# seanwood/gcc-nmf

Measured on AMD Instinct MI355X. Metric: stereo frames/sec (1024-FFT, K=1024, 100 NMF iters), higher is better.
Workload: dtype f32; 1 GPU; HBM-resident (float32 samples in HBM -> separated float32 waveforms in HBM; the host-to-host rates are the host_to_host_* fields of a --full run): 64 x 10 s stereo @16 kHz synthetic mixtures per GPU (SURVEY 8d recipe), 1024-pt FFT hop 256 (F=513, T=622/file), K=1024, 100 KL-NMF iters, 128 TDOAs, 3 targets, independent dictionary per file; dictionary_size=1024, parallelism=file-sharded x1, no data-path collective

## Files before the change

### gcc_nmf_amd/csrc/gemm_dma.h

```cpp
#pragma once
#include <mutex>
#include <type_traits>
#include "gemm_mfma.h"
#include "chain_sync.h"

#ifndef GEMM_DMA_ABL
#define GEMM_DMA_ABL 0
#endif

typedef __attribute__((address_space(3))) void* gemm_lds_ptr;
typedef __attribute__((address_space(1))) const void* gemm_glb_ptr;

__device__ __forceinline__ void gemm_dma16(const float* wave_uniform_base, unsigned lane_byte_offset, unsigned lds_wave_byte_addr) {
    asm volatile("s_mov_b32 m0, %2\n\tglobal_load_lds_dwordx4 %0, %1"
                 :
                 : "v"(lane_byte_offset), "s"(wave_uniform_base), "s"(lds_wave_byte_addr)
                 : "memory");
}

__device__ __forceinline__ void gemm_dma16_masked(const float* wave_uniform_base, unsigned lane_byte_offset, unsigned lds_wave_byte_addr,
                                                  unsigned long long wave_uniform_mask) {
    unsigned long long saved;
    asm volatile("s_mov_b64 %0, exec\n\ts_mov_b64 exec, %4\n\ts_mov_b32 m0, %3\n\tglobal_load_lds_dwordx4 %1, %2\n\ts_mov_b64 exec, %0"
                 : "=&s"(saved)
// ... 8 lines not shown
__device__ __forceinline__ gemm_f32x4 gemm_lds_read_b128(unsigned byte_addr) {
    gemm_f32x4 v;
    asm volatile("ds_read_b128 %0, %1 offset:%2" : "=v"(v) : "v"(byte_addr), "n"(OFF));
    return v;
}
typedef float gemm_f32x2 __attribute__((ext_vector_type(2)));
template <int OFF0, int OFF1>
__device__ __forceinline__ gemm_f32x2 gemm_lds_read2_b32(unsigned byte_addr) {
    gemm_f32x2 v;
    asm volatile("ds_read2_b32 %0, %1 offset0:%2 offset1:%3" : "=v"(v) : "v"(byte_addr), "n"(OFF0), "n"(OFF1));
    return v;
}

__device__ __forceinline__ void gemm_wait_lds() { asm volatile("s_waitcnt lgkmcnt(0)" ::: "memory"); }
template <typename T>
__device__ __forceinline__ void gemm_tie(T& v) { asm volatile("" : "+v"(v)); }

__device__ __forceinline__ void gemm_barrier_arrive(unsigned counter_byte_addr) {
    unsigned long long saved;
    asm volatile("s_mov_b64 %0, exec\n\ts_mov_b64 exec, 1\n\tds_add_u32 %1, %2\n\ts_mov_b64 exec, %0"
                 : "=&s"(saved)
                 : "v"(counter_byte_addr), "v"(1u)
                 : "memory");
}
__device__ __forceinline__ unsigned gemm_barrier_peek(unsigned counter_byte_addr) {
    unsigned seen;
    asm volatile("ds_read_b32 %0, %1" : "=v"(seen) : "v"(counter_byte_addr) : "memory");
    return seen;
}
__device__ __forceinline__ void gemm_barrier_wait(unsigned counter_byte_addr, unsigned target, unsigned seen) {
    unsigned seen_s;
    asm volatile("s_waitcnt lgkmcnt(0)\n1:\n\tv_readfirstlane_b32 %1, %0\n\ts_cmp_ge_u32 %1, %3\n\ts_cbranch_scc1 2f\n\t"
                 "s_sleep 1\n\tds_read_b32 %0, %2\n\ts_waitcnt lgkmcnt(0)\n\ts_branch 1b\n2:"
                 : "+v"(seen), "=&s"(seen_s)
                 : "v"(counter_byte_addr), "s"(target)
                 : "memory", "scc");
}

template <bool KC, int NT, int ROWS>
struct GemmFrag;
template <int NT, int ROWS>
struct GemmFrag<true, NT, ROWS> {
    gemm_f32x4 v[NT];
    __device__ __forceinline__ void read(unsigned base) {
        v[0] = gemm_lds_read_b128<0 * 2048>(base);
        v[1] = gemm_lds_read_b128<1 * 2048>(base);
        if constexpr (NT == 4) {
            v[2] = gemm_lds_read_b128<2 * 2048>(base);
            v[3] = gemm_lds_read_b128<3 * 2048>(base);
        }
    }
    __device__ __forceinline__ void tie() {
// ... 100 lines not shown
                } else {
#pragma unroll
                    for (int r = 0; r < 16; ++r) u[r] = gemm_div_fast(x[r], u[r]);
                }
            }
#pragma unroll
            for (int r = 0; r < 16; ++r) gemm_buffer_store(u[r], C, lane_off, ro + ((r & 3) + 8 * (r >> 2)) * rstep, 0);
        };
        if (oka) column(acc_a, xa, ba, lo);
        if (okb) column(acc_b, xb, bb, lo + 128);
    }
};

template <bool TAIL>
__device__ __forceinline__ void gemm_epilogue_update_w_full(const GemmArgs& p, int file, int col0, int tid, int wm, int l31, int hh,
                                                            bool wave_active, f32x16 (&acc)[4][2], float tail_acc, float rowsum_acc,
                                                            float* smem) {
    float* s_rs = smem;
    float* s_tail = smem + 64;
    float* s_red = smem + 320;
    float* s_norm = smem + 640;
    float rs = rowsum_acc;
    rs += __shfl_xor(rs, 1);
    rs += __shfl_xor(rs, 2);
    if ((tid & 3) == 0) s_rs[tid >> 2] = rs;
    if (TAIL) s_tail[tid] = tail_acc;
    __syncthreads();
    const int ca = l31, cb = l31 + 32;
    const float ira = 1.0f / s_rs[ca], irb = 1.0f / s_rs[cb];
    const gemm_i32x4 W = gemm_buffer_rsrc(p.C + file * p.sC);
    const int lo = 4 * (4 * hh * p.ldc + col0 + l31), rstep = 4 * p.ldc;
    float ssa = 0.f, ssb = 0.f;
    if (wave_active) {
#pragma unroll
        for (int m = 0; m < 4; ++m) {
            const int ro = (wm * 128 + m * 32) * rstep;
            float wa[16], wb[16];
#pragma unroll
            for (int r = 0; r < 16; ++r) {
                const int so = ro + ((r & 3) + 8 * (r >> 2)) * rstep;
// ... 157 lines not shown
        const int r = t - (len + s), base_r = list * p.cr;
        const int lenr = min(max(p.batch * p.rag * p.tiles_m - base_r, 0), p.cr);
        if (r >= lenr) return false;
        const int idx = base_r + r;
        q = idx / p.tiles_m;
        tm = idx - q * p.tiles_m;
        col0 = (p.tiles_n - 1) * 64;
        nw = 1;
    }
    file = gemm_dma_list_file(p, q) + p.file0;
    return true;
}

template <int TM>
struct GemmDmaLds {
    static constexpr int SBUF = 128 * TM * 16 + 64 * 16 + 16 + 16;
};

template <bool A_KC, bool B_KC, int EPI, bool TAIL, int TM, bool NARROW>
__device__ __forceinline__ void gemm_dma_workgroup(const GemmArgs& p, float* const smem, float* const s_rowvec, unsigned* const s_arrivals_p,
                                                   const int list, const int t, const GemmSync& sync, const int sync_it = 0,
                                                   const bool trace_on = true) {
    static_assert(TM == 4 || TM == 2, "");
    static_assert(TM == 4 || EPI != EPI_UPDW, "the fused W update owns all rows of its atoms: full-height tiles only");
    static_assert(!NARROW || (EPI != EPI_UPDW && TM == 4), "narrow items: full-height tiles with an element-wise epilogue");
    constexpr int BK = 16, BM = 128 * TM, BN = 64, RW = 32 * TM;
    constexpr int NA = 2 * TM;
    constexpr int SA = BM * BK, SB = BN * BK;
    constexpr int SBUF = SA + SB + BK + BK;
    static_assert(SBUF == GemmDmaLds<TM>::SBUF, "");
    constexpr bool SCALE = !B_KC && (EPI == EPI_DIV || EPI == EPI_STORE);
    unsigned& s_arrivals = *s_arrivals_p;

    const int tid = threadIdx.x, lane = tid & 63;
    const int wave = __builtin_amdgcn_readfirstlane(tid >> 6);
    const int wm = wave, wn = 0;
    const int l31 = lane & 31, hh = lane >> 5;

    int nkt = (p.Kd + BK - 1) / BK;
    int n_item = p.N;
    int n_sync = p.N;
    int file = 0, tm = 0, col0 = 0, nw = 2, row0 = 0;
    const float* __restrict__ A = nullptr;
    const float* __restrict__ B = nullptr;
    const float* __restrict__ bscale = nullptr;
    const float* __restrict__ tail_src = nullptr;
    const float* __restrict__ scale_src = nullptr;
    unsigned long long tail_mask = 0, scale_mask = 0;
    bool wave_active = false, do_tail = false, do_rowsum = false;
    unsigned offA[NA], offB = 0;
    auto take_item = [&]() -> bool {
        int f_, tm_, c_, nw_;
        if (!gemm_dma_item(p, list, t, f_, tm_, c_, nw_)) return false;
        file = __builtin_amdgcn_readfirstlane(f_);
        tm = __builtin_amdgcn_readfirstlane(tm_);
        col0 = __builtin_amdgcn_readfirstlane(c_);
        nw = NARROW ? __builtin_amdgcn_readfirstlane(nw_) : 2;
        if (p.ragged_n) {
            const int nf = __builtin_amdgcn_readfirstlane(p.ragged_n[file]);
            n_sync = nf;
            if (p.ragged_kd) nkt = (nf + BK - 1) / BK;
            else n_item = nf;
        }
        row0 = tm * BM;
        A = p.A + file * p.sA;
        B = p.B + file * p.sB;
        bscale = (SCALE && p.bscale) ? p.bscale + file * p.s_bscale : nullptr;
        wave_active = (row0 + wm * RW) < p.M;
        do_tail = TAIL && (tm == 0);
        do_rowsum = B_KC && (p.rowsumB != nullptr || EPI == EPI_UPDW) && (tm == 0);
        tail_src = A + (long)p.tail_row * p.lda;
        tail_mask = (wave == 0 && do_tail) ? 0x0full : 0ull;
        scale_mask = (wave == 0 && bscale != nullptr) ? 0xf0ull : 0ull;
        scale_src = bscale != nullptr ? bscale : A;
        return true;
    };
    auto set_offsets = [&]() {
#pragma unroll
        for (int i = 0; i < NA; ++i) {
            const int piece = wave * NA + i;
            if (A_KC) {
                const int row = piece * 16 + (lane >> 2), c = (lane & 3) ^ gemm_swz(piece * 16 + (lane >> 2));
                offA[i] = 4u * (unsigned)(min(row0 + row, p.a_clamp) * p.lda + 4 * c);
            } else {
                constexpr int PPR = BM / 256;
                const int kk = piece / PPR, col = (piece % PPR) * 256 + lane * 4;
                offA[i] = 4u * (unsigned)(kk * p.lda + min(row0 + col, p.a_clamp));
            }
        }
        if (B_KC) {
            const int row = wave * 16 + (lane >> 2), c = (lane & 3) ^ gemm_swz(row);
            offB = 4u * (unsigned)(min(col0 + row, p.b_clamp) * p.ldb + 4 * c);
        } else {
            const int kk = wave * 4 + (lane >> 4), col = (lane & 15) * 4;
            offB = 4u * (unsigned)(kk * p.ldb + min(col0 + col, p.b_clamp));
        }
    };

    f32x16 acc[TM][2];
    float tail_acc = 0.f, rowsum_acc = 0.f;

    const unsigned lds0 = __builtin_amdgcn_readfirstlane((unsigned)(size_t)(gemm_lds_ptr)smem);
    unsigned side_off = 0;

    auto dma_piece = [&](const int piece, const int kt, const int buf) {
#ifdef GEMM_DMA_SKIP_FROM
        if (piece >= GEMM_DMA_SKIP_FROM) return;
#endif
        if (piece < NA) {
            gemm_dma16(A + (A_KC ? (long)kt * BK : (long)kt * BK * p.lda), offA[piece], lds0 + 4 * (buf * SBUF + (wave * NA + piece) * 256));
        } else if (piece == NA) {
            gemm_dma16(B + (B_KC ? (long)kt * BK : (long)kt * BK * p.ldb), offB, lds0 + 4 * (buf * SBUF + SA + wave * 256));
        } else {
            if (TAIL || SCALE) {
                const unsigned dst = lds0 + 4 * (buf * SBUF + SA + SB);
                if (TAIL) gemm_dma16_masked(tail_src + kt * BK, side_off, dst, tail_mask);
                if (SCALE) gemm_dma16_masked(scale_src + kt * BK, side_off, dst, scale_mask);
            }
        }
    };
    constexpr int NPIECES = NA + 2;
#ifdef GEMM_DMA_SPREAD
    constexpr int SPREAD = GEMM_DMA_SPREAD;
#else
    constexpr int SPREAD = (A_KC && !B_KC) ? 1 : 2;
#endif

    const gemm_f32x4 zero4 = {0.f, 0.f, 0.f, 0.f};
    GemmFrag<A_KC, TM, BM> a0, a1;
    GemmFrag<B_KC, 2, BN> b0, b1;
    gemm_f32x4 sc0 = zero4, sc1 = zero4, t4 = zero4, tb4 = zero4, ts4 = zero4, rs4 = zero4;
    gemm_f32x2 tbxy = {0.f, 0.f}, tbzw = {0.f, 0.f};

    const unsigned arrivals_addr = (unsigned)(size_t)(gemm_lds_ptr)s_arrivals_p;
    unsigned oA0 = 0, oA1 = 0, oB0 = 0, oB1 = 0, oTB = 0, oRS = 0;
    const int tg = wave;
    auto set_lane_constants = [&]() {
        const int arow = wm * RW + l31, bcol = wn * 64 + l31, tj = lane;
        side_off = 16u * (unsigned)(lane & 3);
        oA0 = A_KC ? 4 * (arow * 16 + 4 * ((0 + hh) ^ gemm_swz(arow))) : 4 * (4 * (0 + hh) * BM + arow);
        oA1 = A_KC ? 4 * (arow * 16 + 4 * ((2 + hh) ^ gemm_swz(arow))) : 4 * (4 * (2 + hh) * BM + arow);
        oB0 = 4 * SA + (B_KC ? 4 * (bcol * 16 + 4 * ((0 + hh) ^ gemm_swz(bcol))) : 4 * (4 * (0 + hh) * BN + bcol));
        oB1 = 4 * SA + (B_KC ? 4 * (bcol * 16 + 4 * ((2 + hh) ^ gemm_swz(bcol))) : 4 * (4 * (2 + hh) * BN + bcol));
        oTB = 4 * SA + (B_KC ? 4 * (tj * 16 + 4 * (tg ^ gemm_swz(tj))) : 4 * (4 * tg * BN + tj));
        oRS = 4 * SA + 4 * ((tid >> 2) * 16 + 4 * (tid & 3));
    };

    auto read_group0 = [&](const unsigned lds) {
        if (wave_active) {
            a0.read(lds + oA0);
            b0.read(lds + oB0);
        }
        if (SCALE) sc0 = gemm_lds_read_b128<4 * (SA + SB + BK)>(lds + 16 * hh);
    };
    auto read_group1 = [&](const unsigned lds) {
        if (wave_active) {
            a1.read(lds + oA1);
            b1.read(lds + oB1);
        }
        if (SCALE) sc1 = gemm_lds_read_b128<4 * (SA + SB + BK) + 32>(lds + 16 * hh);
        if (TAIL) {
            t4 = gemm_lds_read_b128<4 * (SA + SB)>(lds + 16 * tg);
            if (B_KC) {
                tb4 = gemm_lds_read_b128<0>(lds + oTB);
            } else {
                tbxy = gemm_lds_read2_b32<0 * BN, 1 * BN>(lds + oTB);
                tbzw = gemm_lds_read2_b32<2 * BN, 3 * BN>(lds + oTB);
                if (SCALE) ts4 = gemm_lds_read_b128<4 * (SA + SB + BK)>(lds + 16 * tg);
            }
        }
        if (B_KC) rs4 = gemm_lds_read_b128<0>(lds + oRS);
    };
    auto wait_group0 = [&]() {
        gemm_wait_lds();
        a0.tie();
        b0.tie();
        if (SCALE) {
            gemm_tie(sc0);
            b0.scale(sc0);
        }
    };
    auto wait_group1 = [&]() {
        gemm_wait_lds();
        a1.tie();
        b1.tie();
        if (SCALE) {
            gemm_tie(sc1);
            b1.scale(sc1);
        }
        if (TAIL) {
            gemm_tie(t4);
            if (B_KC) {
                gemm_tie(tb4);
            } else {
                gemm_tie(tbxy);
                gemm_tie(tbzw);
                tb4 = gemm_f32x4{tbxy.x, tbxy.y, tbzw.x, tbzw.y};
                if (SCALE) {
                    gemm_tie(ts4);
                    tb4 *= ts4;
                }
            }
        }
        if (B_KC) gemm_tie(rs4);
    };
    auto mma = [&](auto nw_c, const GemmFrag<A_KC, TM, BM>& a, const GemmFrag<B_KC, 2, BN>& b, const int e, const int m) {
        constexpr int NW = decltype(nw_c)::value;
        acc[m][0] = __builtin_amdgcn_mfma_f32_32x32x2f32(a.get(m, e), b.get(0, e), acc[m][0], 0, 0, 0);
        if constexpr (NW == 2) acc[m][1] = __builtin_amdgcn_mfma_f32_32x32x2f32(a.get(m, e), b.get(1, e), acc[m][1], 0, 0, 0);
    };

#ifdef GEMM_DMA_PROBE
    unsigned long long probe[7] = {0, 0, 0, 0, 0, 0, 0};
#define GEMM_PROBE(i_) const unsigned long long pt##i_ = __builtin_amdgcn_s_memtime()
#define GEMM_PROBE_DECL(i_) unsigned long long pt##i_ = 0
#define GEMM_PROBE_SET(i_) pt##i_ = __builtin_amdgcn_s_memtime()
#else
#define GEMM_PROBE(i_)
#define GEMM_PROBE_DECL(i_)
#define GEMM_PROBE_SET(i_)
#endif
    auto step = [&](auto cur_c, auto nw_c, const int kt) {
        constexpr int CUR = decltype(cur_c)::value;
        const unsigned ldsC = lds0 + 4 * CUR * SBUF, ldsN = lds0 + 4 * (CUR ^ 1) * SBUF;
        const int ktn = min(kt + 1, nkt - 1);
        GEMM_PROBE(0);
#if !(GEMM_DMA_ABL & 1)
        read_group1(ldsC);
#endif
        __builtin_amdgcn_sched_barrier(0);
        if (wave_active) {
            if (SPREAD == 0) {
#pragma unroll
                for (int i = 0; i < NPIECES; ++i) dma_piece(i, ktn, CUR ^ 1);
                __builtin_amdgcn_sched_barrier(0);
            }
#pragma unroll
            for (int e = 0; e < 4; ++e)
#pragma unroll
                for (int m = 0; m < TM; ++m) {
                    mma(nw_c, a0, b0, e, m);
                    const int slot = e * TM + m;
                    if (SPREAD == 1 && slot < NPIECES) {
                        dma_piece(slot, ktn, CUR ^ 1);
                        __builtin_amdgcn_sched_barrier(0);
                    }
                    if (SPREAD == 2 && slot % 3 != 2 && (slot / 3) * 2 + slot % 3 < NPIECES) {
                        dma_piece((slot / 3) * 2 + slot % 3, ktn, CUR ^ 1);
                        __builtin_amdgcn_sched_barrier(0);
                    }
                }
        } else {
#pragma unroll
            for (int i = 0; i < NPIECES; ++i) dma_piece(i, ktn, CUR ^ 1);
        }
        __builtin_amdgcn_sched_barrier(0);
        GEMM_PROBE(1);
        wait_group1();
        GEMM_PROBE(2);
        GEMM_PROBE_DECL(3);
        GEMM_PROBE_DECL(4);
        GEMM_PROBE_DECL(5);
        unsigned seen = 0;
#ifndef GEMM_DMA_ARRIVE_E
#define GEMM_DMA_ARRIVE_E 1
#define GEMM_DMA_WAIT_E 3
#endif
#pragma unroll
        for (int e = 0; e < 4; ++e) {
            if (e == GEMM_DMA_ARRIVE_E) {
                __builtin_amdgcn_sched_barrier(0);
                GEMM_PROBE_SET(3);
                asm volatile("s_waitcnt vmcnt(0)" ::: "memory");
#if !(GEMM_DMA_ABL & 2)
                gemm_barrier_arrive(arrivals_addr);
#endif
                __builtin_amdgcn_sched_barrier(0);
            }
            if (e == GEMM_DMA_WAIT_E - 1) {
                __builtin_amdgcn_sched_barrier(0);
#if !(GEMM_DMA_ABL & 2)
                seen = gemm_barrier_peek(arrivals_addr);
#endif
                __builtin_amdgcn_sched_barrier(0);
            }
            if (e == GEMM_DMA_WAIT_E) {
                __builtin_amdgcn_sched_barrier(0);
                GEMM_PROBE_SET(4);
#if !(GEMM_DMA_ABL & 2)
                gemm_barrier_wait(arrivals_addr, 4u * (unsigned)(kt + 1), seen);
#endif
                GEMM_PROBE_SET(5);
#if !(GEMM_DMA_ABL & 1)
                read_group0(ldsN);
#endif
                __builtin_amdgcn_sched_barrier(0);
            }
            if (wave_active) {
#pragma unroll
                for (int m = 0; m < TM; ++m) mma(nw_c, a1, b1, e, m);
            }
        }
        if (TAIL) {
            tail_acc = fmaf(t4.x, tb4.x, tail_acc);
            tail_acc = fmaf(t4.y, tb4.y, tail_acc);
            tail_acc = fmaf(t4.z, tb4.z, tail_acc);
            tail_acc = fmaf(t4.w, tb4.w, tail_acc);
        }
        if (B_KC) rowsum_acc += (rs4.x + rs4.y) + (rs4.z + rs4.w);
        __builtin_amdgcn_sched_barrier(0);
        GEMM_PROBE(6);
        wait_group0();
#ifdef GEMM_DMA_PROBE
        __builtin_amdgcn_sched_barrier(0);
        const unsigned long long pt7 = __builtin_amdgcn_s_memtime();
        probe[0] += pt1 - pt0;
        probe[1] += pt2 - pt1;
        probe[2] += pt3 - pt2;
        probe[3] += pt4 - pt3;
        probe[4] += pt5 - pt4;
        probe[5] += pt6 - pt5;
        probe[6] += pt7 - pt6;
        __builtin_amdgcn_sched_barrier(0);
#endif
    };
    auto main_loop = [&](auto nw_c) {
        for (int kt = 0; kt < nkt; kt += 2) {
            step(std::integral_constant<int, 0>{}, nw_c, kt);
            if (kt + 1 < nkt) step(std::integral_constant<int, 1>{}, nw_c, kt + 1);
        }
    };

    if (SCALE) {
        if (!p.bscale && tid < 2 * BK) smem[(tid >> 4) * SBUF + SA + SB + BK + (tid & 15)] = 1.f;
    }
    bool have = take_item();
    if (have) set_offsets();
    long long* trace_row = nullptr;
    while (have) {
        const int vb = p.lists == 8 ? 8 * t + list : t;
        trace_row = (trace_on && p.trace && vb < p.trace_rows) ? p.trace + 8 * (long)vb : nullptr;
        if (trace_row && tid == 0) {
            trace_row[0] = trace_row[1] = __builtin_amdgcn_s_memrealtime();
            trace_row[4] = (long long)((__builtin_amdgcn_s_getreg((3 << 11) | 20) & 15u) << 16 | (__builtin_amdgcn_s_getreg((31 << 11) | 4) & 0xffffu));
            trace_row[7] = (long long)blockIdx.x << 16;
        }
        set_lane_constants();
        gemm_sync_wait(sync, file, col0, tid, sync_it, list, n_sync);
        if (trace_row && tid == 0) trace_row[1] = __builtin_amdgcn_s_memrealtime();
#pragma unroll
        for (int i = 0; i < NPIECES; ++i) dma_piece(i, 0, 0);
#pragma unroll
        for (int m = 0; m < TM; ++m)
#pragma unroll
            for (int n = 0; n < 2; ++n)
#pragma unroll
                for (int r = 0; r < 16; ++r) acc[m][n][r] = 0.f;
        tail_acc = 0.f;
        rowsum_acc = 0.f;
        if constexpr (EPI == EPI_STORE || EPI == EPI_UPDH) {
#pragma unroll
            for (int i = 0; i < BM / 256; ++i) {
                const int lr = tid + 256 * i, row = min(row0 + lr, p.M - 1);
                s_rowvec[lr] = p.ktailA ? p.ktailA[file * p.s_ktailA + row] : 0.f;
                if (EPI == EPI_UPDH) {
                    const float rd = 1.0f / (p.E2[file * p.sE2 + row] + p.alpha + p.eps);
                    s_rowvec[BM + lr] = p.E1 ? p.E1[file * p.sE1 + row] * rd : rd;
                }
            }
        }
        if (tid == 0) s_arrivals = 0;
        asm volatile("s_waitcnt vmcnt(0)" ::: "memory");
        __syncthreads();
        read_group0(lds0);
        wait_group0();

        if constexpr (NARROW) {
            if (nw == 1) main_loop(std::integral_constant<int, 1>{});
            else main_loop(std::integral_constant<int, 2>{});
        } else {
            main_loop(std::integral_constant<int, 2>{});
        }
        __syncthreads();
        if (trace_row && tid == 0) trace_row[2] = __builtin_amdgcn_s_memrealtime();

        float* const scratch = smem + SBUF;

        if constexpr (EPI == EPI_UPDW) {
            if constexpr (TM == 4) gemm_epilogue_update_w_full<TAIL>(p, file, col0, tid, wm, l31, hh, wave_active, acc, tail_acc, rowsum_acc, scratch);
        } else {
            if (wave_active) {
                const int row_w = row0 + wm * RW;
                bool lean = false;
                if constexpr (EPI == EPI_STORE || EPI == EPI_DIV || EPI == EPI_UPDH) {
                    lean = row_w + RW <= p.M;
                    if (lean) {
                        GemmEpiloguePair<EPI, BM> e0, e1;
                        const int ca = col0 + l31, tr = wm * RW;
                        const bool oka = ca < n_item, okb = (!NARROW || nw == 2) && ca + 32 < n_item;
                        const long cb = 4L * p.ldc * (p.M + (TAIL ? 1 : 0));
                        float ba = 0.f, bb = 0.f;
                        e0.load(p, file, row_w, hh, ca, cb);
                        e1.load(p, file, row_w + 32, hh, ca, cb);
                        if (EPI != EPI_DIV && p.ktailA) {
// ... 5 lines not shown
                        if constexpr (TM == 4) e0.load(p, file, row_w + 64, hh, ca, cb);
                        e1.finish(p, file, row_w + 32, tr + 32, hh, ca, ba, bb, s_rowvec, acc[1][0], acc[1][1], oka, okb, cb);
                        if constexpr (TM == 4) {
                            e1.load(p, file, row_w + 96, hh, ca, cb);
                            e0.finish(p, file, row_w + 64, tr + 64, hh, ca, ba, bb, s_rowvec, acc[2][0], acc[2][1], oka, okb, cb);
                            e1.finish(p, file, row_w + 96, tr + 96, hh, ca, ba, bb, s_rowvec, acc[3][0], acc[3][1], oka, okb, cb);
                        }
                        if (trace_row && tid == 0) trace_row[6] = __builtin_amdgcn_s_memrealtime();
                    }
                }
                if (!lean) {
                    GemmArgs pq = p;
                    pq.N = n_item;
#pragma unroll
                    for (int m = 0; m < TM; ++m)
                        gemm_epilogue_pair<EPI>(pq, file, row_w + m * 32 + 4 * hh, col0 + wn * 64 + l31, acc[m][0], acc[m][1], !NARROW || nw == 2);
                }
            }
            if (TAIL) {
                if (do_tail) {
                    scratch[tid] = tail_acc;
                    __syncthreads();
                    if (tid < (NARROW && nw == 1 ? 32 : BN)) {
                        const float s = (scratch[tid] + scratch[BN + tid]) + (scratch[2 * BN + tid] + scratch[3 * BN + tid]);
                        const int col = col0 + tid;
                        if (EPI == EPI_PHASE ? gemm_col_valid<EPI>(p, col) : col < n_item) gemm_epilogue<EPI>(p, file, p.tail_row, col, s);
                    }
                }
            }
            if (B_KC) {
                if (do_rowsum) {
                    float s = rowsum_acc;
                    s += __shfl_xor(s, 1);
                    s += __shfl_xor(s, 2);
                    const int j = tid >> 2;
                    if ((tid & 3) == 0 && (col0 + j) < n_item && (!NARROW || nw == 2 || j < 32)) p.rowsumB[file * p.s_rowsumB + col0 + j] = s;
                }
            }
        }
        if (trace_row) {
            asm volatile("s_waitcnt vmcnt(0)" ::: "memory");
            __syncthreads();
            if (tid == 0) trace_row[3] = __builtin_amdgcn_s_memrealtime();
        }
        gemm_sync_signal(sync, file, col0, nw, tid);
        have = false;
    }
#ifdef GEMM_DMA_PROBE
    if (p.trace && lane == 0 && (long)p.trace_grid + 4L * blockIdx.x + 4 <= p.trace_rows) {
#pragma unroll
        for (int i = 0; i < 7; ++i) p.trace[8 * ((long)p.trace_grid + blockIdx.x * 4 + wave) + i] = (long long)probe[i];
        p.trace[8 * ((long)p.trace_grid + blockIdx.x * 4 + wave) + 7] = 1;
    }
#endif
}

template <bool A_KC, bool B_KC, int EPI, bool TAIL, int TM, bool NARROW>
__global__ __launch_bounds__(256, 2) void gccnmf_gemm_dma_kernel(GemmArgs p) {
    __shared__ __attribute__((aligned(16))) float smem[2 * GemmDmaLds<TM>::SBUF];
    __shared__ __attribute__((aligned(16))) float s_rowvec[(EPI == EPI_STORE || EPI == EPI_UPDH) ? 2 * 128 * TM : 4];
    __shared__ unsigned s_arrivals;
    const int list = p.lists == 8 ? (int)(blockIdx.x & 7) : 0;
    const int t = p.lists == 8 ? (int)(blockIdx.x >> 3) : (int)blockIdx.x;
    GemmSync none = {};
    gemm_dma_workgroup<A_KC, B_KC, EPI, TAIL, TM, NARROW>(p, smem, s_rowvec, &s_arrivals, list, t, none);
}

struct GemmChain {
    int first[5];
    int it0, iterations;
    int trace_it;
    GemmSync sync[4];
};
template <bool TAIL, int STAGES, int TM1>
__global__ __launch_bounds__(256, 2) void gccnmf_gemm_chain_kernel(GemmArgs p0, GemmArgs p1, GemmArgs p2, GemmArgs p3, GemmChain ch) {
    static_assert(STAGES == 2 || STAGES == 4, "");
    __shared__ __attribute__((aligned(16))) float smem[2 * GemmDmaLds<4>::SBUF];
    __shared__ __attribute__((aligned(16))) float s_rowvec[2 * 512];
    __shared__ unsigned s_arrivals;
    const int list = (int)(blockIdx.x & 7);
    int pos = (int)(blockIdx.x >> 3), it = ch.it0;
    if (ch.iterations > 1) {
        const int q = pos / ch.first[4];
        it += q;
        pos -= q * ch.first[4];
    }
    const bool tr = it == ch.trace_it;
    if (pos < ch.first[1]) {
        gemm_dma_workgroup<true, false, EPI_DIV, TAIL, 4, true>(p0, smem, s_rowvec, &s_arrivals, list, pos, ch.sync[0], it, tr);
    } else if (pos < ch.first[2]) {
        gemm_dma_workgroup<false, false, EPI_UPDH, false, TM1, TM1 == 4>(p1, smem, s_rowvec, &s_arrivals, list, pos - ch.first[1], ch.sync[1], it, tr);
    } else if constexpr (STAGES == 4) {
        if (pos < ch.first[3]) {
            gemm_dma_workgroup<true, false, EPI_DIV, TAIL, 4, true>(p2, smem, s_rowvec, &s_arrivals, list, pos - ch.first[2], ch.sync[2], it, tr);
        } else {
            gemm_dma_workgroup<true, true, EPI_UPDW, TAIL, 4, false>(p3, smem, s_rowvec, &s_arrivals, list, pos - ch.first[3], ch.sync[3], it, tr);
        }
    }
}

static int gemm_dma_plan(GemmArgs& a, bool narrow_capable, int TM, int whole_files = 0) {
    a.tiles_m = gccnmf_ceil_div(a.M, 128 * TM);
    a.tiles_n = gccnmf_ceil_div(a.N, 64);
    a.lists = (a.xcd_affine && a.batch >= 8) ? 8 : 1;
    const int policy = gccnmf_tune_tail_split;
    const bool narrow_ok = narrow_capable && TM == 4 && policy != 0;
    a.narrow_ok = narrow_ok ? 1 : 0;
    const long tiles = (long)a.batch * a.tiles_m * a.tiles_n;
    if (tiles > (1L << 28)) return -1;
    a.rag = (narrow_ok && a.tiles_n >= 2 && a.N - (a.tiles_n - 1) * 64 <= 32) ? 1 : 0;
    if (a.rag && policy == 1 && !a.concurrent) {
// ... 75 lines not shown
```

Baseline: 155,700 frames/s.

## Load B operand straight into registers and interleave loads across MFMA slots

The B tile is no longer staged through LDS via DMA. Each lane now loads its B fragment directly from global memory into registers, with global loads spread across the inner-loop MFMA slots by a compile-time slot schedule and per-slot vmcnt waits. The A-operand LDS layout for the non-KC case is reorganized per wave, side data (tail/scale) get per-wave LDS slots, and row sums are computed from the register B values. The LDS arrival counter is removed. This aims to cut LDS traffic and per-tile LDS footprint, at the cost of more VGPRs and redundant global B reads across waves, plus tighter hand scheduling that risks stalls if global latency is not hidden.

```diff
diff --git a/gcc_nmf_amd/csrc/gemm_dma.h b/gcc_nmf_amd/csrc/gemm_dma.h
--- a/gcc_nmf_amd/csrc/gemm_dma.h
+++ b/gcc_nmf_amd/csrc/gemm_dma.h
@@ -1,6 +1,7 @@
 #pragma once
 #include <mutex>
 #include <type_traits>
+#include <utility>
 #include "gemm_mfma.h"
 #include "chain_sync.h"
 
@@ -46,28 +47,61 @@
 
 __device__ __forceinline__ void gemm_wait_lds() { asm volatile("s_waitcnt lgkmcnt(0)" ::: "memory"); }
 template <typename T>
-__device__ __forceinline__ void gemm_tie(T& v) { asm volatile("" : "+v"(v)); }
-
-__device__ __forceinline__ void gemm_barrier_arrive(unsigned counter_byte_addr) {
-    unsigned long long saved;
-    asm volatile("s_mov_b64 %0, exec\n\ts_mov_b64 exec, 1\n\tds_add_u32 %1, %2\n\ts_mov_b64 exec, %0"
-                 : "=&s"(saved)
-                 : "v"(counter_byte_addr), "v"(1u)
-                 : "memory");
-}
-__device__ __forceinline__ unsigned gemm_barrier_peek(unsigned counter_byte_addr) {
-    unsigned seen;
-    asm volatile("ds_read_b32 %0, %1" : "=v"(seen) : "v"(counter_byte_addr) : "memory");
-    return seen;
-}
-__device__ __forceinline__ void gemm_barrier_wait(unsigned counter_byte_addr, unsigned target, unsigned seen) {
-    unsigned seen_s;
-    asm volatile("s_waitcnt lgkmcnt(0)\n1:\n\tv_readfirstlane_b32 %1, %0\n\ts_cmp_ge_u32 %1, %3\n\ts_cbranch_scc1 2f\n\t"
-                 "s_sleep 1\n\tds_read_b32 %0, %2\n\ts_waitcnt lgkmcnt(0)\n\ts_branch 1b\n2:"
-                 : "+v"(seen), "=&s"(seen_s)
-                 : "v"(counter_byte_addr), "s"(target)
-                 : "memory", "scc");
-}
+__device__ __forceinline__ void gemm_tie(T& v) { asm volatile("; tie %0" : "+v"(v)); }
+
+template <int OFF>
+__device__ __forceinline__ float gemm_gload(const float* wave_uniform_base, unsigned lane_byte_offset) {
+    float v;
+    asm volatile("s_nop 4\n\tglobal_load_dword %0, %1, %2 offset:%3" : "=v"(v) : "v"(lane_byte_offset), "s"(wave_uniform_base), "n"(OFF) : "memory");
+    return v;
+}
+template <int OFF>
+__device__ __forceinline__ gemm_f32x4 gemm_gload4(const float* wave_uniform_base, unsigned lane_byte_offset) {
+    gemm_f32x4 v;
+    asm volatile("s_nop 4\n\tglobal_load_dwordx4 %0, %1, %2 offset:%3" : "=v"(v) : "v"(lane_byte_offset), "s"(wave_uniform_base), "n"(OFF) : "memory");
+    return v;
+}
+template <int N>
+__device__ __forceinline__ void gemm_wait_vm() {
+    static_assert(N >= 0 && N < 64, "vmcnt is a 6-bit count");
+    asm volatile("s_waitcnt vmcnt(%0)" : : "n"(N) : "memory");
+}
+template <typename F, int... I>
+__device__ __forceinline__ void gemm_static_for_impl(F&& f, std::integer_sequence<int, I...>) { (f(std::integral_constant<int, I>{}), ...); }
+template <int N, typename F>
+__device__ __forceinline__ void gemm_static_for(F&& f) { gemm_static_for_impl(f, std::make_integer_sequence<int, N>{}); }
+
+template <bool B_KC, int TM, int NMISC>
+struct GemmDmaSlots {
+    static constexpr int NSLOT = 8 * TM;
+    static constexpr int BSPAN = B_KC ? 4 * TM : TM;
+    static constexpr bool b_slot(int s) { return s % BSPAN == BSPAN - 1; }
+    static constexpr int nonb_before(int s) {
+        int n = 0;
+        for (int i = 0; i < s; ++i) n += b_slot(i) ? 0 : 1;
+        return n;
+    }
+    static constexpr int per() { const int window = nonb_before(NSLOT) * 5 / 8; return (NMISC + window - 1) / window; }
+    static constexpr int misc_first(int s) { return per() * nonb_before(s); }
+    static constexpr int ops(int s) {
+        if (b_slot(s)) return 2;
+        const int left = NMISC - misc_first(s);
+        return left < 0 ? 0 : left > per() ? per() : left;
+    }
+    static constexpr int ops_in(int s0, int s1) {
+        int n = 0;
+        for (int s = s0; s < s1; ++s) n += ops(s);
+        return n;
+    }
+    static constexpr int total() { return ops_in(0, NSLOT); }
+    static constexpr int b_pending(int s0) { return total() - ops_in(s0, s0 + BSPAN); }
+    static constexpr int misc_pending(int s) {
+        int last = -1;
+        for (int i = 0; i < NSLOT; ++i)
+            if (!b_slot(i) && ops(i) > 0) last = i;
+        return ops_in(last + 1, s);
+    }
+};
 
 template <bool KC, int NT, int ROWS>
 struct GemmFrag;
@@ -198,16 +232,16 @@
 
 template <bool TAIL>
 __device__ __forceinline__ void gemm_epilogue_update_w_full(const GemmArgs& p, int file, int col0, int tid, int wm, int l31, int hh,
-                                                            bool wave_active, f32x16 (&acc)[4][2], float tail_acc, float rowsum_acc,
-                                                            float* smem) {
+                                                            bool wave_active, f32x16 (&acc)[4][2], float tail_acc, float rowsum_a,
+                                                            float rowsum_b, float* smem) {
     float* s_rs = smem;
     float* s_tail = smem + 64;
     float* s_red = smem + 320;
     float* s_norm = smem + 640;
-    float rs = rowsum_acc;
-    rs += __shfl_xor(rs, 1);
-    rs += __shfl_xor(rs, 2);
-    if ((tid & 3) == 0) s_rs[tid >> 2] = rs;
+    if (tid < 32) {
+        s_rs[tid] = rowsum_a;
+        s_rs[tid + 32] = rowsum_b;
+    }
     if (TAIL) s_tail[tid] = tail_acc;
     __syncthreads();
     const int ca = l31, cb = l31 + 32;
@@ -395,11 +429,12 @@
 
 template <int TM>
 struct GemmDmaLds {
-    static constexpr int SBUF = 128 * TM * 16 + 64 * 16 + 16 + 16;
+    static constexpr int SIDE = 16 + 16 + 16;
+    static constexpr int SBUF = 128 * TM * 16 + 4 * SIDE;
 };
 
 template <bool A_KC, bool B_KC, int EPI, bool TAIL, int TM, bool NARROW>
-__device__ __forceinline__ void gemm_dma_workgroup(const GemmArgs& p, float* const smem, float* const s_rowvec, unsigned* const s_arrivals_p,
+__device__ __forceinline__ void gemm_dma_workgroup(const GemmArgs& p, float* const smem, float* const s_rowvec,
                                                    const int list, const int t, const GemmSync& sync, const int sync_it = 0,
                                                    const bool trace_on = true) {
     static_assert(TM == 4 || TM == 2, "");
@@ -407,15 +442,18 @@
     static_assert(!NARROW || (EPI != EPI_UPDW && TM == 4), "narrow items: full-height tiles with an element-wise epilogue");
     constexpr int BK = 16, BM = 128 * TM, BN = 64, RW = 32 * TM;
     constexpr int NA = 2 * TM;
-    constexpr int SA = BM * BK, SB = BN * BK;
-    constexpr int SBUF = SA + SB + BK + BK;
+    constexpr int SA = BM * BK, SIDE = GemmDmaLds<TM>::SIDE;
+    constexpr int SBUF = SA + 4 * SIDE;
     static_assert(SBUF == GemmDmaLds<TM>::SBUF, "");
     constexpr bool SCALE = !B_KC && (EPI == EPI_DIV || EPI == EPI_STORE);
-    unsigned& s_arrivals = *s_arrivals_p;
+    constexpr int NTB = TAIL ? (B_KC ? 1 : 4) : 0, NS = (TAIL ? 1 : 0) + (SCALE ? 1 : 0), NMISC = NTB + NS + NA;
+    typedef GemmDmaSlots<B_KC, TM, NMISC> SL;
+    constexpr int NSLOT = SL::NSLOT;
+    static_assert(SL::total() < 64 && SL::misc_pending(7 * TM) >= 0 && SL::misc_first(7 * TM) >= NMISC, "");
 
     const int tid = threadIdx.x, lane = tid & 63;
     const int wave = __builtin_amdgcn_readfirstlane(tid >> 6);
-    const int wm = wave, wn = 0;
+    const int wm = wave;
     const int l31 = lane & 31, hh = lane >> 5;
 
     int nkt = (p.Kd + BK - 1) / BK;
@@ -427,9 +465,9 @@
     const float* __restrict__ bscale = nullptr;
     const float* __restrict__ tail_src = nullptr;
     const float* __restrict__ scale_src = nullptr;
-    unsigned long long tail_mask = 0, scale_mask = 0;
+    unsigned scale_sink = 0;
     bool wave_active = false, do_tail = false, do_rowsum = false;
-    unsigned offA[NA], offB = 0;
+    unsigned offA[NA], offB[2] = {0, 0}, offT = 0;
     auto take_item = [&]() -> bool {
         int f_, tm_, c_, nw_;
         if (!gemm_dma_item(p, list, t, f_, tm_, c_, nw_)) return false;
@@ -451,156 +489,153 @@
         do_tail = TAIL && (tm == 0);
         do_rowsum = B_KC && (p.rowsumB != nullptr || EPI == EPI_UPDW) && (tm == 0);
         tail_src = A + (long)p.tail_row * p.lda;
-        tail_mask = (wave == 0 && do_tail) ? 0x0full : 0ull;
-        scale_mask = (wave == 0 && bscale != nullptr) ? 0xf0ull : 0ull;
         scale_src = bscale != nullptr ? bscale : A;
+        scale_sink = bscale != nullptr ? 0u : 64u;
         return true;
     };
     auto set_offsets = [&]() {
 #pragma unroll
         for (int i = 0; i < NA; ++i) {
-            const int piece = wave * NA + i;
             if (A_KC) {
-                const int row = piece * 16 + (lane >> 2), c = (lane & 3) ^ gemm_swz(piece * 16 + (lane >> 2));
+                const int row = (wave * NA + i) * 16 + (lane >> 2), c = (lane & 3) ^ gemm_swz(row);
                 offA[i] = 4u * (unsigned)(min(row0 + row, p.a_clamp) * p.lda + 4 * c);
             } else {
-                constexpr int PPR = BM / 256;
-                const int kk = piece / PPR, col = (piece % PPR) * 256 + lane * 4;
+                constexpr int LPR = RW / 4;
+                const int kk = i * (64 / LPR) + lane / LPR, col = wave * RW + (lane % LPR) * 4;
                 offA[i] = 4u * (unsigned)(kk * p.lda + min(row0 + col, p.a_clamp));
             }
         }
-        if (B_KC) {
-            const int row = wave * 16 + (lane >> 2), c = (lane & 3) ^ gemm_swz(row);
-            offB = 4u * (unsigned)(min(col0 + row, p.b_clamp) * p.ldb + 4 * c);
-        } else {
-            const int kk = wave * 4 + (lane >> 4), col = (lane & 15) * 4;
-            offB = 4u * (unsigned)(kk * p.ldb + min(col0 + col, p.b_clamp));
-        }
+        auto bcol = [&](const int j) { return min(j & ~3, p.b_clamp) + (j & 3); };
+#pragma unroll
+        for (int c = 0; c < 2; ++c) {
+            if (B_KC) offB[c] = 4u * (unsigned)(min(col0 + 32 * c + l31, p.b_clamp) * p.ldb + 4 * hh);
+            else offB[c] = 4u * (unsigned)(4 * hh * p.ldb + bcol(col0 + 32 * c + l31));
+        }
+        if (TAIL) offT = B_KC ? 4u * (unsigned)(min(col0 + lane, p.b_clamp) * p.ldb) : 4u * (unsigned)bcol(col0 + lane);
     };
 
     f32x16 acc[TM][2];
-    float tail_acc = 0.f, rowsum_acc = 0.f;
+    float tail_acc = 0.f;
+    float rowsum_acc[2][2] = {{0.f, 0.f}, {0.f, 0.f}};
 
     const unsigned lds0 = __builtin_amdgcn_readfirstlane((unsigned)(size_t)(gemm_lds_ptr)smem);
     unsigned side_off = 0;
 
-    auto dma_piece = [&](const int piece, const int kt, const int buf) {
-#ifdef GEMM_DMA_SKIP_FROM
-        if (piece >= GEMM_DMA_SKIP_FROM) return;
-#endif
-        if (piece < NA) {
-            gemm_dma16(A + (A_KC ? (long)kt * BK : (long)kt * BK * p.lda), offA[piece], lds0 + 4 * (buf * SBUF + (wave * NA + piece) * 256));
-        } else if (piece == NA) {
-            gemm_dma16(B + (B_KC ? (long)kt * BK : (long)kt * BK * p.ldb), offB, lds0 + 4 * (buf * SBUF + SA + wave * 256));
+    auto dma_a = [&](const int i, const int kt, const int buf) {
+        gemm_dma16(A + (A_KC ? (long)kt * BK : (long)kt * BK * p.lda), offA[i], lds0 + 4 * (buf * SBUF + (wave * NA + i) * 256));
+    };
+    auto dma_side = [&](const int i, const int kt, const int buf) {
+        const unsigned dst = lds0 + 4 * (buf * SBUF + SA + wave * SIDE);
+        if (TAIL && i == 0) gemm_dma16_masked(tail_src + kt * BK, side_off, dst, 0x0full);
+        else gemm_dma16_masked(scale_src + kt * BK, side_off, dst + scale_sink, 0xf0ull);
+    };
+
+    float bf[2][4][2] = {};
+    gemm_f32x4 bv[2][2] = {};
+    auto load_b = [&](auto q_c, auto e_c, const int kt) {
+        constexpr int q = decltype(q_c)::value, e = decltype(e_c)::value;
+        if constexpr (B_KC) {
+            bv[q][0] = gemm_gload4<32 * q>(B + (long)kt * BK, offB[0]);
+            bv[q][1] = gemm_gload4<32 * q>(B + (long)kt * BK, offB[1]);
         } else {
-            if (TAIL || SCALE) {
-                const unsigned dst = lds0 + 4 * (buf * SBUF + SA + SB);
-                if (TAIL) gemm_dma16_masked(tail_src + kt * BK, side_off, dst, tail_mask);
-                if (SCALE) gemm_dma16_masked(scale_src + kt * BK, side_off, dst, scale_mask);
-            }
-        }
-    };
-    constexpr int NPIECES = NA + 2;
-#ifdef GEMM_DMA_SPREAD
-    constexpr int SPREAD = GEMM_DMA_SPREAD;
-#else
-    constexpr int SPREAD = (A_KC && !B_KC) ? 1 : 2;
-#endif
+            const float* row = B + ((long)kt * BK + 8 * q + e) * p.ldb;
+            bf[q][e][0] = gemm_gload<0>(row, offB[0]);
+            bf[q][e][1] = gemm_gload<0>(row, offB[1]);
+        }
+    };
+    float tbf[4] = {0.f, 0.f, 0.f, 0.f};
+    gemm_f32x4 tb4 = {0.f, 0.f, 0.f, 0.f};
+    auto load_tb = [&](auto i_c, const int kt) {
+        constexpr int i = decltype(i_c)::value;
+        if constexpr (B_KC) tb4 = gemm_gload4<0>(B + (long)kt * BK + 4 * wave, offT);
+        else tbf[i] = gemm_gload<0>(B + ((long)kt * BK + 4 * wave + i) * p.ldb, offT);
+    };
+    auto issue_misc = [&](auto j_c, const int kt, const int ktn, const int buf) {
+        constexpr int j = decltype(j_c)::value;
+        if constexpr (j < NTB) load_tb(j_c, kt);
+        else if constexpr (j < NTB + NS) dma_side(j - NTB, ktn, buf);
+        else dma_a(j - NTB - NS, ktn, buf);
+    };
 
     const gemm_f32x4 zero4 = {0.f, 0.f, 0.f, 0.f};
-    GemmFrag<A_KC, TM, BM> a0, a1;
-    GemmFrag<B_KC, 2, BN> b0, b1;
-    gemm_f32x4 sc0 = zero4, sc1 = zero4, t4 = zero4, tb4 = zero4, ts4 = zero4, rs4 = zero4;
-    gemm_f32x2 tbxy = {0.f, 0.f}, tbzw = {0.f, 0.f};
-
-    const unsigned arrivals_addr = (unsigned)(size_t)(gemm_lds_ptr)s_arrivals_p;
-    unsigned oA0 = 0, oA1 = 0, oB0 = 0, oB1 = 0, oTB = 0, oRS = 0;
+    GemmFrag<A_KC, TM, RW> a0, a1;
+    gemm_f32x4 sc0 = zero4, sc1 = zero4, t4 = zero4, ts4 = zero4;
+
+    unsigned oA0 = 0, oA1 = 0, oSh = 0, oSt = 0;
     const int tg = wave;
     auto set_lane_constants = [&]() {
-        const int arow = wm * RW + l31, bcol = wn * 64 + l31, tj = lane;
+        const int arow = wm * RW + l31;
         side_off = 16u * (unsigned)(lane & 3);
-        oA0 = A_KC ? 4 * (arow * 16 + 4 * ((0 + hh) ^ gemm_swz(arow))) : 4 * (4 * (0 + hh) * BM + arow);
-        oA1 = A_KC ? 4 * (arow * 16 + 4 * ((2 + hh) ^ gemm_swz(arow))) : 4 * (4 * (2 + hh) * BM + arow);
-        oB0 = 4 * SA + (B_KC ? 4 * (bcol * 16 + 4 * ((0 + hh) ^ gemm_swz(bcol))) : 4 * (4 * (0 + hh) * BN + bcol));
-        oB1 = 4 * SA + (B_KC ? 4 * (bcol * 16 + 4 * ((2 + hh) ^ gemm_swz(bcol))) : 4 * (4 * (2 + hh) * BN + bcol));
-        oTB = 4 * SA + (B_KC ? 4 * (tj * 16 + 4 * (tg ^ gemm_swz(tj))) : 4 * (4 * tg * BN + tj));
-        oRS = 4 * SA + 4 * ((tid >> 2) * 16 + 4 * (tid & 3));
+        oA0 = A_KC ? 4 * (arow * 16 + 4 * ((0 + hh) ^ gemm_swz(arow))) : 4 * (wm * RW * 16 + 4 * (0 + hh) * RW + l31);
+        oA1 = A_KC ? 4 * (arow * 16 + 4 * ((2 + hh) ^ gemm_swz(arow))) : 4 * (wm * RW * 16 + 4 * (2 + hh) * RW + l31);
+        oSh = 4 * (SA + wave * SIDE) + 16 * hh;
+        oSt = 4 * (SA + wave * SIDE) + 16 * tg;
     };
 
     auto read_group0 = [&](const unsigned lds) {
-        if (wave_active) {
-            a0.read(lds + oA0);
-            b0.read(lds + oB0);
-        }
-        if (SCALE) sc0 = gemm_lds_read_b128<4 * (SA + SB + BK)>(lds + 16 * hh);
+        if (wave_active) a0.read(lds + oA0);
+        if (SCALE) sc0 = gemm_lds_read_b128<64>(lds + oSh);
     };
     auto read_group1 = [&](const unsigned lds) {
-        if (wave_active) {
-            a1.read(lds + oA1);
-            b1.read(lds + oB1);
-        }
-        if (SCALE) sc1 = gemm_lds_read_b128<4 * (SA + SB + BK) + 32>(lds + 16 * hh);
+        if (wave_active) a1.read(lds + oA1);
+        if (SCALE) sc1 = gemm_lds_read_b128<64 + 32>(lds + oSh);
         if (TAIL) {
-            t4 = gemm_lds_read_b128<4 * (SA + SB)>(lds + 16 * tg);
-            if (B_KC) {
-                tb4 = gemm_lds_read_b128<0>(lds + oTB);
-            } else {
-                tbxy = gemm_lds_read2_b32<0 * BN, 1 * BN>(lds + oTB);
-                tbzw = gemm_lds_read2_b32<2 * BN, 3 * BN>(lds + oTB);
-                if (SCALE) ts4 = gemm_lds_read_b128<4 * (SA + SB + BK)>(lds + 16 * tg);
-            }
-        }
-        if (B_KC) rs4 = gemm_lds_read_b128<0>(lds + oRS);
+            t4 = gemm_lds_read_b128<0>(lds + oSt);
+            if (SCALE) ts4 = gemm_lds_read_b128<64>(lds + oSt);
+        }
     };
     auto wait_group0 = [&]() {
         gemm_wait_lds();
         a0.tie();
-        b0.tie();
-        if (SCALE) {
-            gemm_tie(sc0);
-            b0.scale(sc0);
-        }
+        if (SCALE) gemm_tie(sc0);
     };
     auto wait_group1 = [&]() {
         gemm_wait_lds();
         a1.tie();
-        b1.tie();
-        if (SCALE) {
-            gemm_tie(sc1);
-            b1.scale(sc1);
-        }
+        if (SCALE) gemm_tie(sc1);
         if (TAIL) {
             gemm_tie(t4);
-            if (B_KC) {
-                gemm_tie(tb4);
+            if (SCALE) gemm_tie(ts4);
+        }
+    };
+    auto need_b = [&](auto q_c, auto e_c) {
+        constexpr int q = decltype(q_c)::value, e = decltype(e_c)::value;
+        gemm_wait_vm<SL::b_pending((4 * q + e) * TM)>();
+#pragma unroll
+        for (int c = 0; c < 2; ++c) {
+            if constexpr (B_KC) {
+                gemm_tie(bv[q][c]);
+                rowsum_acc[q][c] += (bv[q][c].x + bv[q][c].y) + (bv[q][c].z + bv[q][c].w);
             } else {
-                gemm_tie(tbxy);
-                gemm_tie(tbzw);
-                tb4 = gemm_f32x4{tbxy.x, tbxy.y, tbzw.x, tbzw.y};
-                if (SCALE) {
-                    gemm_tie(ts4);
-                    tb4 *= ts4;
-                }
-            }
-        }
-        if (B_KC) gemm_tie(rs4);
-    };
-    auto mma = [&](auto nw_c, const GemmFrag<A_KC, TM, BM>& a, const GemmFrag<B_KC, 2, BN>& b, const int e, const int m) {
+                gemm_tie(bf[q][e][c]);
+                if (SCALE) bf[q][e][c] *= q == 0 ? sc0[e] : sc1[e];
+            }
+        }
+    };
+    auto mma = [&](auto nw_c, const GemmFrag<A_KC, TM, RW>& a, const int q, const int e, const int m) {
         constexpr int NW = decltype(nw_c)::value;
-        acc[m][0] = __builtin_amdgcn_mfma_f32_32x32x2f32(a.get(m, e), b.get(0, e), acc[m][0], 0, 0, 0);
-        if constexpr (NW == 2) acc[m][1] = __builtin_amdgcn_mfma_f32_32x32x2f32(a.get(m, e), b.get(1, e), acc[m][1], 0, 0, 0);
+        acc[m][0] = __builtin_amdgcn_mfma_f32_32x32x2f32(a.get(m, e), B_KC ? bv[q][0][e] : bf[q][e][0], acc[m][0], 0, 0, 0);
+        if constexpr (NW == 2) acc[m][1] = __builtin_amdgcn_mfma_f32_32x32x2f32(a.get(m, e), B_KC ? bv[q][1][e] : bf[q][e][1], acc[m][1], 0, 0, 0);
     };
 
 #ifdef GEMM_DMA_PROBE
     unsigned long long probe[7] = {0, 0, 0, 0, 0, 0, 0};
 #define GEMM_PROBE(i_) const unsigned long long pt##i_ = __builtin_amdgcn_s_memtime()
-#define GEMM_PROBE_DECL(i_) unsigned long long pt##i_ = 0
-#define GEMM_PROBE_SET(i_) pt##i_ = __builtin_amdgcn_s_memtime()
 #else
 #define GEMM_PROBE(i_)
-#define GEMM_PROBE_DECL(i_)
-#define GEMM_PROBE_SET(i_)
 #endif
+    auto slot = [&](auto s_c, auto nw_c, const int kt, const int ktn, const int nbuf) {
+        constexpr int S = decltype(s_c)::value, q = S / (4 * TM), e = (S / TM) & 3, m = S % TM;
+        constexpr std::integral_constant<int, q> q_c{};
+        constexpr std::integral_constant<int, e> e_c{};
+        if constexpr (m == 0 && (!B_KC || e == 0)) need_b(q_c, e_c);
+        if constexpr (q == 0) mma(nw_c, a0, q, e, m);
+        else mma(nw_c, a1, q, e, m);
+        __builtin_amdgcn_sched_barrier(0);
+        if constexpr (SL::b_slot(S)) load_b(q_c, e_c, ktn);
+        else gemm_static_for<SL::ops(S)>([&](auto k_c) { issue_misc(std::integral_constant<int, SL::misc_first(S) + decltype(k_c)::value>{}, kt, ktn, nbuf); });
+        __builtin_amdgcn_sched_barrier(0);
+    };
     auto step = [&](auto cur_c, auto nw_c, const int kt) {
         constexpr int CUR = decltype(cur_c)::value;
         const unsigned ldsC = lds0 + 4 * CUR * SBUF, ldsN = lds0 + 4 * (CUR ^ 1) * SBUF;
@@ -611,97 +646,51 @@
 #endif
         __builtin_amdgcn_sched_barrier(0);
         if (wave_active) {
-            if (SPREAD == 0) {
-#pragma unroll
-                for (int i = 0; i < NPIECES; ++i) dma_piece(i, ktn, CUR ^ 1);
-                __builtin_amdgcn_sched_barrier(0);
-            }
-#pragma unroll
-            for (int e = 0; e < 4; ++e)
-#pragma unroll
-                for (int m = 0; m < TM; ++m) {
-                    mma(nw_c, a0, b0, e, m);
-                    const int slot = e * TM + m;
-                    if (SPREAD == 1 && slot < NPIECES) {
-                        dma_piece(slot, ktn, CUR ^ 1);
-                        __builtin_amdgcn_sched_barrier(0);
-                    }
-                    if (SPREAD == 2 && slot % 3 != 2 && (slot / 3) * 2 + slot % 3 < NPIECES) {
-                        dma_piece((slot / 3) * 2 + slot % 3, ktn, CUR ^ 1);
-                        __builtin_amdgcn_sched_barrier(0);
-                    }
-                }
-        } else {
-#pragma unroll
-            for (int i = 0; i < NPIECES; ++i) dma_piece(i, ktn, CUR ^ 1);
+            gemm_static_for<NSLOT / 2>([&](auto i_c) { slot(i_c, nw_c, kt, ktn, CUR ^ 1); });
+        } else if (TAIL) {
+            gemm_static_for<NTB + NS>([&](auto j_c) { issue_misc(j_c, kt, ktn, CUR ^ 1); });
         }
         __builtin_amdgcn_sched_barrier(0);
         GEMM_PROBE(1);
         wait_group1();
         GEMM_PROBE(2);
-        GEMM_PROBE_DECL(3);
-        GEMM_PROBE_DECL(4);
-        GEMM_PROBE_DECL(5);
-        unsigned seen = 0;
-#ifndef GEMM_DMA_ARRIVE_E
-#define GEMM_DMA_ARRIVE_E 1
-#define GEMM_DMA_WAIT_E 3
+        if (wave_active) gemm_static_for<3 * TM>([&](auto i_c) { slot(std::integral_constant<int, NSLOT / 2 + decltype(i_c)::value>{}, nw_c, kt, ktn, CUR ^ 1); });
+        __builtin_amdgcn_sched_barrier(0);
+        GEMM_PROBE(3);
+        if (wave_active) gemm_wait_vm<SL::misc_pending(7 * TM)>();
+        else gemm_wait_vm<0>();
+        GEMM_PROBE(4);
+#if !(GEMM_DMA_ABL & 1)
+        read_group0(ldsN);
 #endif
-#pragma unroll
-        for (int e = 0; e < 4; ++e) {
-            if (e == GEMM_DMA_ARRIVE_E) {
-                __builtin_amdgcn_sched_barrier(0);
-                GEMM_PROBE_SET(3);
-                asm volatile("s_waitcnt vmcnt(0)" ::: "memory");
-#if !(GEMM_DMA_ABL & 2)
-                gemm_barrier_arrive(arrivals_addr);
-#endif
-                __builtin_amdgcn_sched_barrier(0);
-            }
-            if (e == GEMM_DMA_WAIT_E - 1) {
-                __builtin_amdgcn_sched_barrier(0);
-#if !(GEMM_DMA_ABL & 2)
-                seen = gemm_barrier_peek(arrivals_addr);
-#endif
-                __builtin_amdgcn_sched_barrier(0);
-            }
-            if (e == GEMM_DMA_WAIT_E) {
-                __builtin_amdgcn_sched_barrier(0);
-                GEMM_PROBE_SET(4);
-#if !(GEMM_DMA_ABL & 2)
-                gemm_barrier_wait(arrivals_addr, 4u * (unsigned)(kt + 1), seen);
-#endif
-                GEMM_PROBE_SET(5);
-#if !(GEMM_DMA_ABL & 1)
-                read_group0(ldsN);
-#endif
-                __builtin_amdgcn_sched_barrier(0);
-            }
-            if (wave_active) {
-#pragma unroll
-                for (int m = 0; m < TM; ++m) mma(nw_c, a1, b1, e, m);
-            }
-        }
+        __builtin_amdgcn_sched_barrier(0);
+        if (wave_active) gemm_static_for<TM>([&](auto i_c) { slot(std::integral_constant<int, 7 * TM + decltype(i_c)::value>{}, nw_c, kt, ktn, CUR ^ 1); });
         if (TAIL) {
+            if (B_KC) {
+                gemm_tie(tb4);
+            } else {
+#pragma unroll
+                for (int i = 0; i < 4; ++i) gemm_tie(tbf[i]);
+                tb4 = gemm_f32x4{tbf[0], tbf[1], tbf[2], tbf[3]};
+                if (SCALE) tb4 *= ts4;
+            }
             tail_acc = fmaf(t4.x, tb4.x, tail_acc);
             tail_acc = fmaf(t4.y, tb4.y, tail_acc);
             tail_acc = fmaf(t4.z, tb4.z, tail_acc);
             tail_acc = fmaf(t4.w, tb4.w, tail_acc);
         }
-        if (B_KC) rowsum_acc += (rs4.x + rs4.y) + (rs4.z + rs4.w);
         __builtin_amdgcn_sched_barrier(0);
-        GEMM_PROBE(6);
+        GEMM_PROBE(5);
         wait_group0();
 #ifdef GEMM_DMA_PROBE
         __builtin_amdgcn_sched_barrier(0);
-        const unsigned long long pt7 = __builtin_amdgcn_s_memtime();
+        const unsigned long long pt6 = __builtin_amdgcn_s_memtime();
         probe[0] += pt1 - pt0;
         probe[1] += pt2 - pt1;
         probe[2] += pt3 - pt2;
         probe[3] += pt4 - pt3;
         probe[4] += pt5 - pt4;
         probe[5] += pt6 - pt5;
-        probe[6] += pt7 - pt6;
         __builtin_amdgcn_sched_barrier(0);
 #endif
     };
@@ -713,8 +702,12 @@
     };
 
     if (SCALE) {
-        if (!p.bscale && tid < 2 * BK) smem[(tid >> 4) * SBUF + SA + SB + BK + (tid & 15)] = 1.f;
-    }
+        if (!p.bscale && tid < 128) smem[(tid >> 6) * SBUF + SA + ((tid >> 4) & 3) * SIDE + BK + (tid & 15)] = 1.f;
+    }
+    auto row_sum = [&](const int c) {
+        const float u0 = rowsum_acc[0][c] + __shfl_xor(rowsum_acc[0][c], 32), u1 = rowsum_acc[1][c] + __shfl_xor(rowsum_acc[1][c], 32);
+        return u0 + u1;
+    };
     bool have = take_item();
     if (have) set_offsets();
     long long* trace_row = nullptr;
@@ -729,8 +722,18 @@
         set_lane_constants();
         gemm_sync_wait(sync, file, col0, tid, sync_it, list, n_sync);
         if (trace_row && tid == 0) trace_row[1] = __builtin_amdgcn_s_memrealtime();
-#pragma unroll
-        for (int i = 0; i < NPIECES; ++i) dma_piece(i, 0, 0);
+        if (wave_active || TAIL) {
+#pragma unroll
+            for (int i = 0; i < NS; ++i) dma_side(i, 0, 0);
+        }
+        float b_touch = 0.f;
+        if (wave_active) {
+#pragma unroll
+            for (int i = 0; i < NA; ++i) dma_a(i, 0, 0);
+            const unsigned line = B_KC ? 4u * (unsigned)(min(col0 + lane, p.b_clamp) * p.ldb)
+                                       : 4u * (unsigned)((lane >> 2) * p.ldb + min(col0 + 16 * (lane & 3), p.b_clamp));
+            b_touch = gemm_gload<0>(B, line);
+        }
 #pragma unroll
         for (int m = 0; m < TM; ++m)
 #pragma unroll
@@ -738,7 +741,7 @@
 #pragma unroll
                 for (int r = 0; r < 16; ++r) acc[m][n][r] = 0.f;
         tail_acc = 0.f;
-        rowsum_acc = 0.f;
+        rowsum_acc[0][0] = rowsum_acc[0][1] = rowsum_acc[1][0] = rowsum_acc[1][1] = 0.f;
         if constexpr (EPI == EPI_STORE || EPI == EPI_UPDH) {
 #pragma unroll
             for (int i = 0; i < BM / 256; ++i) {
@@ -750,8 +753,30 @@
                 }
             }
         }
-        if (tid == 0) s_arrivals = 0;
-        asm volatile("s_waitcnt vmcnt(0)" ::: "memory");
+        auto land_b = [&]() {
+            gemm_wait_vm<0>();
+#pragma unroll
+            for (int q = 0; q < 2; ++q)
+#pragma unroll
+                for (int c = 0; c < 2; ++c) {
+                    if constexpr (B_KC) {
+                        gemm_tie(bv[q][c]);
+                    } else {
+#pragma unroll
+                        for (int e = 0; e < 4; ++e) gemm_tie(bf[q][e][c]);
+                    }
+                }
+        };
+        __builtin_amdgcn_sched_barrier(0);
+        if (wave_active) {
+            gemm_static_for<8>([&](auto i_c) {
+                constexpr int i = decltype(i_c)::value;
+                if constexpr (!B_KC || (i & 3) == 3) load_b(std::integral_constant<int, i / 4>{}, std::integral_constant<int, i & 3>{}, 0);
+            });
+        }
+        land_b();
+        gemm_tie(b_touch);
+        __builtin_amdgcn_sched_barrier(0);
         __syncthreads();
         read_group0(lds0);
         wait_group0();
@@ -762,13 +787,17 @@
         } else {
             main_loop(std::integral_constant<int, 2>{});
         }
+        land_b();
         __syncthreads();
         if (trace_row && tid == 0) trace_row[2] = __builtin_amdgcn_s_memrealtime();
 
         float* const scratch = smem + SBUF;
 
         if constexpr (EPI == EPI_UPDW) {
-            if constexpr (TM == 4) gemm_epilogue_update_w_full<TAIL>(p, file, col0, tid, wm, l31, hh, wave_active, acc, tail_acc, rowsum_acc, scratch);
+            if constexpr (TM == 4) {
+                const float rs_a = row_sum(0), rs_b = row_sum(1);
+                gemm_epilogue_update_w_full<TAIL>(p, file, col0, tid, wm, l31, hh, wave_active, acc, tail_acc, rs_a, rs_b, scratch);
+            }
         } else {
             if (wave_active) {
                 const int row_w = row0 + wm * RW;
@@ -804,7 +833,7 @@
                     pq.N = n_item;
 #pragma unroll
                     for (int m = 0; m < TM; ++m)
-                        gemm_epilogue_pair<EPI>(pq, file, row_w + m * 32 + 4 * hh, col0 + wn * 64 + l31, acc[m][0], acc[m][1], !NARROW || nw == 2);
+                        gemm_epilogue_pair<EPI>(pq, file, row_w + m * 32 + 4 * hh, col0 + l31, acc[m][0], acc[m][1], !NARROW || nw == 2);
                 }
             }
             if (TAIL) {
@@ -820,11 +849,11 @@
             }
             if (B_KC) {
                 if (do_rowsum) {
-                    float s = rowsum_acc;
-                    s += __shfl_xor(s, 1);
-                    s += __shfl_xor(s, 2);
-                    const int j = tid >> 2;
-                    if ((tid & 3) == 0 && (col0 + j) < n_item && (!NARROW || nw == 2 || j < 32)) p.rowsumB[file * p.s_rowsumB + col0 + j] = s;
+                    const float rs_a = row_sum(0), rs_b = row_sum(1);
+                    if (tid < 32) {
+                        if (col0 + tid < n_item) p.rowsumB[file * p.s_rowsumB + col0 + tid] = rs_a;
+                        if (col0 + tid + 32 < n_item && (!NARROW || nw == 2)) p.rowsumB[file * p.s_rowsumB + col0 + tid + 32] = rs_b;
+                    }
                 }
             }
         }
@@ -849,11 +878,10 @@
 __global__ __launch_bounds__(256, 2) void gccnmf_gemm_dma_kernel(GemmArgs p) {
     __shared__ __attribute__((aligned(16))) float smem[2 * GemmDmaLds<TM>::SBUF];
     __shared__ __attribute__((aligned(16))) float s_rowvec[(EPI == EPI_STORE || EPI == EPI_UPDH) ? 2 * 128 * TM : 4];
-    __shared__ unsigned s_arrivals;
     const int list = p.lists == 8 ? (int)(blockIdx.x & 7) : 0;
     const int t = p.lists == 8 ? (int)(blockIdx.x >> 3) : (int)blockIdx.x;
     GemmSync none = {};
-    gemm_dma_workgroup<A_KC, B_KC, EPI, TAIL, TM, NARROW>(p, smem, s_rowvec, &s_arrivals, list, t, none);
+    gemm_dma_workgroup<A_KC, B_KC, EPI, TAIL, TM, NARROW>(p, smem, s_rowvec, list, t, none);
 }
 
 struct GemmChain {
@@ -867,7 +895,6 @@
     static_assert(STAGES == 2 || STAGES == 4, "");
     __shared__ __attribute__((aligned(16))) float smem[2 * GemmDmaLds<4>::SBUF];
     __shared__ __attribute__((aligned(16))) float s_rowvec[2 * 512];
-    __shared__ unsigned s_arrivals;
     const int list = (int)(blockIdx.x & 7);
     int pos = (int)(blockIdx.x >> 3), it = ch.it0;
     if (ch.iterations > 1) {
@@ -877,14 +904,14 @@
     }
     const bool tr = it == ch.trace_it;
     if (pos < ch.first[1]) {
-        gemm_dma_workgroup<true, false, EPI_DIV, TAIL, 4, true>(p0, smem, s_rowvec, &s_arrivals, list, pos, ch.sync[0], it, tr);
+        gemm_dma_workgroup<true, false, EPI_DIV, TAIL, 4, true>(p0, smem, s_rowvec, list, pos, ch.sync[0], it, tr);
     } else if (pos < ch.first[2]) {
-        gemm_dma_workgroup<false, false, EPI_UPDH, false, TM1, TM1 == 4>(p1, smem, s_rowvec, &s_arrivals, list, pos - ch.first[1], ch.sync[1], it, tr);
+        gemm_dma_workgroup<false, false, EPI_UPDH, false, TM1, TM1 == 4>(p1, smem, s_rowvec, list, pos - ch.first[1], ch.sync[1], it, tr);
     } else if constexpr (STAGES == 4) {
         if (pos < ch.first[3]) {
-            gemm_dma_workgroup<true, false, EPI_DIV, TAIL, 4, true>(p2, smem, s_rowvec, &s_arrivals, list, pos - ch.first[2], ch.sync[2], it, tr);
+            gemm_dma_workgroup<true, false, EPI_DIV, TAIL, 4, true>(p2, smem, s_rowvec, list, pos - ch.first[2], ch.sync[2], it, tr);
         } else {
-            gemm_dma_workgroup<true, true, EPI_UPDW, TAIL, 4, false>(p3, smem, s_rowvec, &s_arrivals, list, pos - ch.first[3], ch.sync[3], it, tr);
+            gemm_dma_workgroup<true, true, EPI_UPDW, TAIL, 4, false>(p3, smem, s_rowvec, list, pos - ch.first[3], ch.sync[3], it, tr);
         }
     }
 }
```

Measured after the change: 153,900 frames/s. 1.2% lower.
